# InternetMaximalism/plonky2_bn254

Measured on AMD Instinct MI355X. Metric: G1 scalar-mul STARK proofs/sec (256-bit scalars), higher is better.
Workload: dtype u64 (Goldilocks p = 2^64-2^32+1; BN254 Fq as 10x26-bit Montgomery limbs); 1 GPU; configs[1]: batch of 1024 G1 scalar-muls on 1 GPU per step = 8 proofs x 128 instances, 2^16 rows, W=781, standard_fast_config; instances_per_proof=128, steps_in_flight=4, parallelism=1 GPU, no collective

## Files before the change

include/bn254_stark.h:

```cpp
#ifndef BN254_STARK_H
#define BN254_STARK_H

#include <stddef.h>
#include <stdint.h>

#ifdef __cplusplus
extern "C" {
#endif

#define BN254S_ABI_VERSION 1

enum {
  BN254S_OK = 0,
  BN254S_E_INVALID_ARG = -1,
  BN254S_E_HIP = -2,
  BN254S_E_OOM = -3,
  BN254S_E_INVALID_POINT = -4,
  BN254S_E_UNSUPPORTED = -5,
  BN254S_E_TRANSCRIPT = -6,
  BN254S_E_INTERNAL = -7,
  BN254S_E_VERIFY = -8
};

typedef struct bn254s_ctx bn254s_ctx;
// ... 143 lines not shown
int bn254s_job_outputs_batch(bn254s_ctx* ctx, int kind, const uint64_t* scalars , const uint64_t* x,
                             const uint64_t* offset, size_t n, uint64_t* outputs_out ,
                             uint8_t* finite_out );
int bn254s_job_outputs(bn254s_ctx* ctx, int kind, const bn254s_params* params, const uint64_t* scalars, const uint64_t* x,
                       const uint64_t* offset, size_t n, size_t per_proof, uint64_t* outputs_out, bn254s_proof** proofs_out);
int bn254s_commit_values(bn254s_ctx* ctx, const uint64_t* values, size_t ncols, uint64_t* coeffs, uint64_t* lde,
                         uint64_t* cap);
int bn254s_bench_ntt(bn254s_ctx* ctx, size_t ncols, int iters, float* ms);
int bn254s_bench_ntt_clock(bn254s_ctx* ctx, size_t ncols, int iters, float* ms, float* mhz, float* mhz_min);
int bn254s_bench_issue(bn254s_ctx* ctx, float* ns_per_issue, float* mhz);
int bn254s_bench_copy(bn254s_ctx* ctx, size_t words, int iters);
int bn254s_bench_leafhash(bn254s_ctx* ctx, size_t ncols, int log_leaves, int iters, float* ms);
int bn254s_poseidon_permute(bn254s_ctx* ctx, uint64_t* states, size_t n);
int bn254s_selftest_field(bn254s_ctx* ctx, const uint64_t* a, const uint64_t* b, size_t n, uint64_t* out);
int bn254s_selftest_poseidon(bn254s_ctx* ctx, int variant, uint64_t* states, size_t n);
int bn254s_selftest_leaf_hash(bn254s_ctx* ctx, const uint64_t* data, size_t ncols, int log_leaves, int kernel, int chunk_cols,
                              uint64_t* digests);
int bn254s_selftest_fq_inv(bn254s_ctx* ctx, const uint64_t* x, size_t n, uint64_t* out);
int bn254s_selftest_fq(bn254s_ctx* ctx, int group, const uint64_t* in, size_t n, uint64_t* out);
int bn254s_selftest_logup(bn254s_ctx* ctx, const uint64_t* trace, size_t rows, int ncols, int rc_begin, int n_rc, int table_col,
                          int freq_col, const uint64_t betas[2], uint64_t* out);
int bn254s_selftest_acc(bn254s_ctx* ctx, const uint64_t* values, const uint64_t* weights, size_t T, size_t rows, uint64_t* out);
int bn254s_selftest_openings(bn254s_ctx* ctx, const uint64_t* coeffs, int npolys, int log_r, const uint64_t zeta[2],
                             const uint64_t zeta_next[2], uint64_t* out);
int bn254s_selftest_fri_combine(bn254s_ctx* ctx, int mode, int W, int n_rc, int n_ctl, size_t n, const uint64_t* cols,
                                const uint64_t* aux_in, const uint64_t* points, uint64_t* out);
int bn254s_selftest_fri_fold(bn254s_ctx* ctx, const uint64_t* in, int log_m, uint64_t shift, const uint64_t beta[2], uint64_t* out);
int bn254s_selftest_fri_rows(bn254s_ctx* ctx, const uint64_t* lde, int ncols, int log_n, int h, size_t k0, size_t rows,
                             const uint32_t* indices, int nq, uint64_t* window, uint64_t* gathered);
int bn254s_selftest_transforms(bn254s_ctx* ctx, int op, int log_n, int flags, int ncols, int coset_mask, const uint64_t* in,
                               uint64_t* out0, uint64_t* out1);
int bn254s_selftest_mul_2exp(bn254s_ctx* ctx, const uint64_t* x, size_t n, uint64_t* out);
int bn254s_selftest_outer_dft(bn254s_ctx* ctx, int log_r, int inverse, const uint64_t* in, size_t n, uint64_t* out);
#define BN254S_VERIFY_RECORD_HEAD 34
int bn254s_selftest_verify_front(int kind, const bn254s_params* params, uint32_t degree_bits, const uint64_t* words, size_t n_words,
                                 uint64_t* record_out, size_t record_cap);
int bn254s_selftest_query_round(bn254s_ctx* ctx, int kind, const bn254s_params* params, uint32_t degree_bits,
                                const uint64_t* const* words, size_t n_words, const uint64_t* records, size_t n_proofs,
                                size_t chunk_proofs, int32_t* codes_out);
const char* bn254s_selftest_query_text(int n_layers, int code);
int bn254s_selftest_verify_batch_ms(bn254s_ctx* ctx, float ms_out[5]);
#define BN254S_PLAN_WORDS 54
int bn254s_selftest_proof_plan(int kind, size_t n, const bn254s_params* params, uint64_t dev_total_bytes, int force_split,
                               int force_lowmem, int force_stream, int stream_win_log, uint64_t* out, char* err, size_t err_len);
int bn254s_generate_trace(bn254s_ctx* ctx, int kind, const uint64_t* scalars, const uint64_t* x, const uint64_t* offset,
                          size_t n, uint32_t min_rows_log2, uint64_t* trace_out, uint64_t* outputs);
int bn254s_g1_generate_trace(bn254s_ctx* ctx, const uint64_t* scalars, const uint64_t* x, const uint64_t* offset,
                             size_t n, uint32_t min_rows_log2, uint64_t* trace_out, uint64_t* outputs);

#ifdef __cplusplus
}
#endif
#endif
```

plonky2_bn254_amd/csrc/ctx.h:

```cpp
#pragma once
#include <string>
#include <vector>
#include <map>
#include <cstdio>
#include <mutex>
#include <condition_variable>
#include <chrono>
#include <deque>
#include <functional>
#include <thread>
#include <atomic>
#include <hip/hip_runtime.h>
#include "../../include/bn254_stark.h"
#include "gl_dev.h"
#include "ntt.h"

struct BufPool {
  std::map<std::string, std::pair<void*, size_t>> pool;
  std::string err;
  void* buf(const std::string& name, size_t bytes) {
    auto it = pool.find(name);
    if (it != pool.end() && it->second.second >= bytes) return it->second.first;
    if (it != pool.end()) {
      hipFree(it->second.first);
      pool.erase(it);
    }
    void* p = nullptr;
    if (hipMalloc(&p, bytes) != hipSuccess) {
      (void)hipGetLastError();
      err = "hipMalloc failed for " + name + " (" + std::to_string(bytes) + " bytes)";
      return nullptr;
    }
    pool[name] = {p, bytes};
    return p;
  }
  u64* words(const std::string& name, size_t n) { return (u64*)buf(name, n * 8); }
  bool has(const std::string& name) const { return pool.find(name) != pool.end(); }
  void drop(const std::string& name) {
    auto it = pool.find(name);
    if (it == pool.end()) return;
    hipFree(it->second.first);
    pool.erase(it);
  }
  void release() {
    for (auto& kv : pool) hipFree(kv.second.first);
    pool.clear();
  }
};

struct Slot {
  hipStream_t st = nullptr;
  BufPool mem;
  void* pinned = nullptr;
  size_t pinned_bytes = 0;
  std::vector<hipEvent_t> events;
};

enum { BIG_NTT = 0, BIG_EXCL = 1, BIG_HASH = 2, BIG_HASH_PART = 3 };

struct WorkPool {
  std::mutex mu;
  std::condition_variable cv, done_cv;
  std::deque<std::function<void(size_t)>> q;
  std::vector<std::thread> th;
  std::vector<char> busy;
  bool stop = false;
  size_t limit = 0, n_busy = 0;
  size_t n_waiting = 0, completions = 0;
  std::mutex retry_mu;
  std::atomic<int> in_flight{0};
  void start(size_t n, int device) {
    std::lock_guard<std::mutex> lk(mu);
    limit = n;
    if (busy.size() < n) busy.resize(n, 0);
    while (th.size() < n) {
      th.emplace_back([this, device]() {
        (void)hipSetDevice(device);
        for (;;) {
          std::function<void(size_t)> f;
          size_t s = 0;
          {
            std::unique_lock<std::mutex> lk2(mu);
            auto free_slot = [&]() -> size_t {
              for (size_t i = 0; i < limit && i < busy.size(); i++)
                if (!busy[i]) return i;
              return (size_t)-1;
            };
            cv.wait(lk2, [&] { return (stop && q.empty()) || (!q.empty() && n_busy < limit && free_slot() != (size_t)-1); });
            if (q.empty()) return;
            f = std::move(q.front());
            q.pop_front();
// ... 36 lines not shown
    }
    for (size_t i : idle) g(i);
    {
      std::lock_guard<std::mutex> lk(mu);
      for (size_t i : idle) busy[i] = 0;
    }
    cv.notify_all();
  }
  size_t active() {
    std::lock_guard<std::mutex> lk(mu);
    return n_busy - n_waiting;
  }
  size_t completions_now() {
    std::lock_guard<std::mutex> lk(mu);
    return completions;
  }
  void wait_for_a_completion(size_t c0) {
    std::unique_lock<std::mutex> lk(mu);
    n_waiting++;
    done_cv.wait_for(lk, std::chrono::seconds(60), [&] { return completions != c0; });
    n_waiting--;
  }
  void shutdown() {
    {
      std::lock_guard<std::mutex> lk(mu);
      stop = true;
    }
    cv.notify_all();
    for (auto& t : th) t.join();
    th.clear();
  }
};

struct bn254s_ctx : BufPool {
  int device = 0;
  hipStream_t stream = nullptr;
  NttTables ntt;
  std::vector<Slot*> slots;
  WorkPool workers;
  std::mutex plans_mu;
  std::map<std::pair<unsigned, bool>, NttPlan> plans;
  const NttPlan* ntt_plan(unsigned log_n, bool split) {
    std::lock_guard<std::mutex> lk(plans_mu);
    const auto key = std::make_pair(log_n, split);
    auto it = plans.find(key);
    if (it != plans.end()) return &it->second;
    NttPlan p;
    if (ntt_plan_init(&p, &ntt, log_n, split) != 0) return nullptr;
    return &(plans[key] = p);
  }
  std::mutex big_mu;
  std::condition_variable big_cv;
  int big_cap = 12, big_cost[4] = {12, 2, 4, 2}, big_used = 0;
  int hash_split = 1;
  bool big_fifo = true;
  struct BigWaiter {
    unsigned long id;
    int cls;
  };
  std::deque<BigWaiter> big_q;
  unsigned long big_next_id = 0;
  int big_convoy = 4, big_convoy_run = 0;
  bool big_last_was_ntt = false;
  void big_lock(int cls) {
    std::unique_lock<std::mutex> lk(big_mu);
    if (big_fifo) {
      const unsigned long my = big_next_id++;
      big_q.push_back({my, cls});
      big_cv.wait(lk, [&] {
        if (big_q.front().id == my) {
          if (big_used + big_cost[cls] > big_cap) return false;
          if (big_last_was_ntt && cls != BIG_NTT && big_convoy_run < big_convoy)
            for (const BigWaiter& w : big_q)
              if (w.cls == BIG_NTT) return false;
          return true;
        }
        if (cls != BIG_NTT || !big_last_was_ntt || big_used != 0 || big_convoy_run >= big_convoy) return false;
        if (big_q.front().cls == BIG_NTT) return false;
        for (const BigWaiter& w : big_q) {
          if (w.cls == BIG_NTT) return w.id == my;
        }
        return false;
      });
      const bool in_order = big_q.front().id == my;
      for (auto it = big_q.begin(); it != big_q.end(); ++it)
        if (it->id == my) {
          big_q.erase(it);
          break;
        }
      if (in_order) big_convoy_run = 0;
      else big_convoy_run++;
      big_last_was_ntt = false;
      big_used += big_cost[cls];
      lk.unlock();
      big_cv.notify_all();
      return;
    }
    big_cv.wait(lk, [&] { return big_used + big_cost[cls] <= big_cap; });
    big_used += big_cost[cls];
  }
  void big_unlock(int cls) {
    {
      std::lock_guard<std::mutex> lk(big_mu);
      big_used -= big_cost[cls];
      big_last_was_ntt = cls == BIG_NTT && big_used == 0;
    }
    big_cv.notify_all();
  }
  static constexpr size_t MAX_SLOTS = 64;
  std::mutex slots_mu, err_mu;
  float vb_ms[5] = {0, 0, 0, 0, 0};
  bn254s_ctx() { slots.reserve(MAX_SLOTS); }
  void set_err(const std::string& e) {
    std::lock_guard<std::mutex> lk(err_mu);
    err = e;
  }
  size_t n_slots_now() {
    std::lock_guard<std::mutex> lk(slots_mu);
    return slots.size();
  }
  Slot* slot(size_t i) {
    if (i >= MAX_SLOTS) return nullptr;
    std::lock_guard<std::mutex> lk(slots_mu);
    while (slots.size() <= i) {
      Slot* s = new Slot();
      if (hipStreamCreateWithFlags(&s->st, hipStreamNonBlocking) != hipSuccess) {
        delete s;
        return nullptr;
      }
      slots.push_back(s);
    }
    return slots[i];
  }
};

#define HIP_TRY(ctx, call)                                                                  \
  do {                                                                                      \
    hipError_t e_ = (call);                                                                 \
    if (e_ != hipSuccess) {                                                                 \
      (ctx)->set_err(std::string(#call) + ": " + hipGetErrorString(e_));                    \
      return BN254S_E_HIP;                                                                  \
// ... 3 lines not shown
```

plonky2_bn254_amd/csrc/ntt.h:

```cpp
#pragma once
#include <vector>
#include "gl_dev.h"

static constexpr size_t NTT_N = 65536;

struct NttTables {
  u64 *tw256_fwd = nullptr, *tw256_inv = nullptr;
  u64 *twmat_fwd = nullptr, *twmat_inv = nullptr;
  u64* twmat_inv_ninv = nullptr;
  u64* coset_pow[2] = {nullptr, nullptr};
  u64* coset_inv_pow[2] = {nullptr, nullptr};
  u64 n_inv = 0;
};

int ntt_tables_init(NttTables* T);
void ntt_tables_free(NttTables* T);

struct NttTallTables {
  unsigned log_n = 0;
  u64* wn_inv_pow = nullptr;
  u64* wn_pow_br = nullptr;
  u64* block_coset_pow[2] = {nullptr, nullptr};
  u64 shift[2] = {0, 0};
  u64 r_inv = 0;
};
struct NttSplitTables {
  unsigned log_n = 0;
  u64 *fwd_lo = nullptr, *fwd_hi = nullptr, *inv_lo = nullptr, *inv_hi = nullptr;
  u64 shift[2] = {0, 0};
  u64 half = 0;
};

struct NttPlan {
  unsigned log_n = 0, log_s = 0, log_r = 0;
  const NttTables* base = nullptr;
  NttTallTables tall;
  NttSplitTables split;
};
int ntt_plan_init(NttPlan* P, const NttTables* base, unsigned log_n, bool split);
void ntt_plan_free(NttPlan* P);
size_t ntt_scratch_words(unsigned log_n, bool split, int ncols);
void ntt_commit(const NttPlan& P, const u64* vals, u64* coef, u64* lde, size_t lde_stride, u64* scratch, int ncols, hipStream_t s);
void ntt_lde(const NttPlan& P, const u64* coef, u64* lde, size_t lde_stride, u64* scratch, int ncols, hipStream_t s, int coset_mask = 3);
void ntt_coset_inverse(const NttPlan& P, int h, const u64* vals, u64* coef, u64* scratch, int ncols, hipStream_t s);

static constexpr int FIELD_SELFTEST_OUTS = 17;
void field_selftest(const u64* a, const u64* b, u64* out, size_t n, hipStream_t s);
void mul_2exp_selftest(const u64* x, u64* out, size_t n, hipStream_t s);
void outer_dft_selftest(int log_r, bool inverse, const u64* in, u64* out, size_t n, hipStream_t s);
```

plonky2_bn254_amd/csrc/ntt.hip:

```cpp
#include <cassert>
#include <type_traits>
#include "gl_dev.h"
#include "gl_asm.h"
#include "ntt.h"

#if defined(__HIP_DEVICE_COMPILE__) && defined(BN254S_NTT_PRIO) && BN254S_NTT_PRIO > 0
#define NTT_KERNEL_PRIO() __builtin_amdgcn_s_setprio(BN254S_NTT_PRIO)
#else
#define NTT_KERNEL_PRIO() ((void)0)
#endif

template <bool INV, int SPAN, int G, int J>
__device__ __forceinline__ void bfly16(u64* x) {
  constexpr int E = J * (8 / SPAN);
  constexpr int S0 = E == 0 ? 0 : (!INV ? 12 * E : 192 - 12 * E);
  constexpr bool NEG0 = S0 >= 96;
  constexpr int S1 = NEG0 ? S0 - 96 : S0;
  constexpr bool RIGHT = S1 > 64;
  constexpr bool NEG = NEG0 != RIGHT;
  u64 s, d;
  gl_bfly_asm<NEG>(x[G + J], x[G + J + SPAN], s, d);
  x[G + J] = s;
  if constexpr (S1 == 0) x[G + J + SPAN] = d;
  else if constexpr (RIGHT) x[G + J + SPAN] = gl_shr_small_asm<96 - S1>(d);
// ... 618 lines not shown
  k_coset_unscale_half<<<dim3((unsigned)(H / 256), 2 * ncols), 256, 0, s>>>(coeffs, H, TT->log_n - 16, gl_mul(si, si));
}

int ntt_plan_init(NttPlan* P, const NttTables* base, unsigned log_n, bool split) {
  *P = NttPlan{};
  if (log_n < 16 || log_n - split > 22 || (split && log_n < 18)) return -1;
  P->log_n = log_n;
  P->log_s = split ? 1 : 0;
  P->log_r = log_n - 16 - P->log_s;
  P->base = base;
  if ((P->log_r && tall_tables_init(&P->tall, log_n - P->log_s, split ? gl_mul(GL_GEN, GL_GEN) : GL_GEN)) ||
      (split && split_tables_init(&P->split, log_n))) {
    ntt_plan_free(P);
    return -1;
  }
  return 0;
}
void ntt_plan_free(NttPlan* P) {
  tall_tables_free(&P->tall);
  split_tables_free(&P->split);
}
size_t ntt_scratch_words(unsigned log_n, bool split, int ncols) { return (size_t)(log_n == 16 || split ? 3 : 1) * ncols << log_n; }

void ntt_commit(const NttPlan& P, const u64* vals, u64* coef, u64* lde, size_t lde_stride, u64* scratch, int ncols, hipStream_t s) {
  const size_t N = (size_t)1 << P.log_n;
  assert(P.log_s || lde_stride == 2 * N);
  if (P.log_s) {
    split_inverse(&P.split, vals, coef, ncols, s);
    commit_tall(P.base, &P.tall, coef, coef, scratch, scratch + (size_t)ncols * 2 * N, 2 * ncols, s);
    split_forward(&P.split, scratch, lde, lde_stride, ncols, s, 3);
  } else if (P.log_r) commit_tall(P.base, &P.tall, vals, coef, lde, scratch, ncols, s);
  else commit_base(P.base, vals, coef, lde, scratch, ncols, s);
}
void ntt_lde(const NttPlan& P, const u64* coef, u64* lde, size_t lde_stride, u64* scratch, int ncols, hipStream_t s, int coset_mask) {
  const size_t N = (size_t)1 << P.log_n;
  assert(P.log_s || lde_stride == 2 * N);
  assert(P.log_r || coset_mask == 3);
  if (P.log_s) {
    lde_tall(P.base, &P.tall, coef, scratch, scratch + (size_t)ncols * 2 * N, 2 * ncols, s, coset_mask);
    split_forward(&P.split, scratch, lde, lde_stride, ncols, s, coset_mask);
  } else if (P.log_r) lde_tall(P.base, &P.tall, coef, lde, scratch, ncols, s, coset_mask);
  else lde_base(P.base, coef, lde, scratch, ncols, s);
}
void ntt_coset_inverse(const NttPlan& P, int h, const u64* vals, u64* coef, u64* scratch, int ncols, hipStream_t s) {
  if (P.log_s) coset_inverse_split(P.base, &P.tall, &P.split, h, vals, coef, scratch, ncols, s);
  else if (P.log_r) coset_inverse_tall(P.base, &P.tall, h, vals, coef, scratch, ncols, s);
  else coset_inverse_base(P.base, h, vals, coef, scratch, ncols, s);
}

__global__ void k_field_selftest(const u64* __restrict__ a, const u64* __restrict__ b, u64* __restrict__ out, size_t n) {
  size_t i = (size_t)blockIdx.x * blockDim.x + threadIdx.x;
  if (i >= n) return;
  const u64 x = a[i], y = b[i];
  u64* o = out + i * FIELD_SELFTEST_OUTS;
  u64 s, d, s2, d2;
  gl_bfly_asm<false>(x, y, s, d);
  gl_bfly_asm<true>(x, y, s2, d2);
  o[0] = s;
  o[1] = d;
  o[2] = d2;
  o[3] = s2 == s ? gl_mul_asm(x, y) : ~0ull;
  o[4] = gl_shl_asm<12>(x);
  o[5] = gl_shl_asm<24>(x);
  o[6] = gl_shl_asm<32>(x);
  o[7] = gl_shl_asm<36>(x);
  o[8] = gl_shl_asm<48>(x);
// ... 49 lines not shown
```

plonky2_bn254_amd/csrc/ntt_selftest.hip:

```cpp
#include "ctx.h"
#include "transforms.h"

static bool all_canonical(const uint64_t* w, size_t n) {
  for (size_t k = 0; k < n; k++)
    if (w[k] >= GL_P) return false;
  return true;
}

extern "C" {

int bn254s_selftest_transforms(bn254s_ctx* c, int op, int log_n, int flags, int ncols, int coset_mask, const uint64_t* in,
                               uint64_t* out0, uint64_t* out1) {
  if (!c || !in || !out0 || (op == 0 && !out1)) return BN254S_E_INVALID_ARG;
  if (op < 0 || op > 3 || log_n < 16 || log_n > 23 || flags < 0 || flags > 3 || ncols < 1 || ncols > 64) return BN254S_E_INVALID_ARG;
  const bool split = flags & 1, compact = flags & 2;
  if ((split && log_n < 18) || (!split && log_n == 23) || (compact && log_n == 16)) return BN254S_E_INVALID_ARG;
  if (op == 2 && (log_n == 16 || ncols > Transforms::CH || coset_mask < 1 || coset_mask > 3)) return BN254S_E_INVALID_ARG;
  if (op == 3 && ncols != 2 * 2) return BN254S_E_INVALID_ARG;
  if (op == 1 && compact && !split && ncols > Transforms::CH) return BN254S_E_INVALID_ARG;
  ProofPlan pl;
  pl.log_n = (unsigned)log_n;
  const size_t N = pl.N = (size_t)1 << log_n, M2 = pl.M2 = 2 * N;
  pl.log_m2 = pl.log_n + 1;
  pl.log_s = split ? 1 : 0;
// ... 2 lines not shown
  if (!all_canonical(in, n_in)) return BN254S_E_INVALID_ARG;

  HIP_TRY(c, hipSetDevice(c->device));
  const NttPlan* np = c->ntt_plan(pl.log_n, split);
  if (!np) {
    c->set_err("NTT tables");
    return BN254S_E_OOM;
  }
  const size_t n_lde = (size_t)ncols * M2;
  u64* d_in = c->words("ns.in", n_in);
  u64* d_coef = op == 0 || op == 3 ? c->words("ns.coef", n_in) : nullptr;
  u64* d_lde = op != 3 ? c->words("ns.lde", n_lde) : nullptr;
  u64* d_tmp = c->words("ns.tmp", pl.ntt_tmp_words(ncols));
  if (!d_in || !d_tmp || (!d_coef && (op == 0 || op == 3)) || (!d_lde && op != 3)) return BN254S_E_OOM;
  hipStream_t st = c->stream;
  HIP_TRY(c, hipMemcpyAsync(d_in, in, 8 * n_in, hipMemcpyHostToDevice, st));
  const Transforms tf{*np, st, pl, d_tmp, d_lde, nullptr};
  switch (op) {
    case 0: tf.commit_ntt(d_in, d_coef, d_lde, ncols); break;
    case 1: tf.lde(d_in, d_lde, ncols); break;
    case 2:
      HIP_TRY(c, hipMemsetAsync(d_lde, 0xFF, 8 * n_lde, st));
      tf.lde_chunk(d_in, ncols, coset_mask);
      break;
    default: tf.quotient_coset_inverse(d_in, d_coef); break;
  }
  HIP_TRY(c, hipGetLastError());
  if (op == 0 || op == 3) HIP_TRY(c, hipMemcpyAsync(out0, d_coef, 8 * n_in, hipMemcpyDeviceToHost, st));
  if (op != 3) HIP_TRY(c, hipMemcpyAsync(op == 0 ? out1 : out0, d_lde, 8 * n_lde, hipMemcpyDeviceToHost, st));
  HIP_TRY(c, hipStreamSynchronize(st));
  return BN254S_OK;
}

int bn254s_selftest_mul_2exp(bn254s_ctx* c, const uint64_t* x, size_t n, uint64_t* out) {
  if (!c || !x || !out || n < 1 || n > ((size_t)1 << 20) || !all_canonical(x, n)) return BN254S_E_INVALID_ARG;
  HIP_TRY(c, hipSetDevice(c->device));
  u64* d = c->words("ns.shift", n + 64 * n);
  if (!d) return BN254S_E_OOM;
  HIP_TRY(c, hipMemcpyAsync(d, x, 8 * n, hipMemcpyHostToDevice, c->stream));
  mul_2exp_selftest(d, d + n, n, c->stream);
  HIP_TRY(c, hipGetLastError());
  HIP_TRY(c, hipMemcpyAsync(out, d + n, 8 * 64 * n, hipMemcpyDeviceToHost, c->stream));
  HIP_TRY(c, hipStreamSynchronize(c->stream));
  return BN254S_OK;
}

int bn254s_selftest_outer_dft(bn254s_ctx* c, int log_r, int inverse, const uint64_t* in, size_t n, uint64_t* out) {
  if (!c || !in || !out || log_r < 1 || log_r > 6 || inverse < 0 || inverse > 1 || n < 1 || n > ((size_t)1 << 16)) return BN254S_E_INVALID_ARG;
  const size_t words = n << log_r;
  if (!all_canonical(in, words)) return BN254S_E_INVALID_ARG;
  HIP_TRY(c, hipSetDevice(c->device));
  u64* d = c->words("ns.dft", 2 * words);
  if (!d) return BN254S_E_OOM;
  HIP_TRY(c, hipMemcpyAsync(d, in, 8 * words, hipMemcpyHostToDevice, c->stream));
  outer_dft_selftest(log_r, inverse != 0, d, d + words, n, c->stream);
  HIP_TRY(c, hipGetLastError());
  HIP_TRY(c, hipMemcpyAsync(out, d + words, 8 * words, hipMemcpyDeviceToHost, c->stream));
  HIP_TRY(c, hipStreamSynchronize(c->stream));
  return BN254S_OK;
}

}
```

plonky2_bn254_amd/csrc/prover.hip:

```cpp
#include <algorithm>
#include <atomic>
#include <cstring>
#include <thread>
#include "ctx.h"
#include "trace.h"
#include "aux.h"
#include "merkle.h"
#include "quotient.h"
#include "fri.h"
#include "transcript.h"
#include "prover.h"
#include "proof_plan.h"
#include "transforms.h"

template <class L>
static StarkShape make_shape(bool input_has_a, int n_constraints) {
  StarkShape s;
  s.W = L::W;
  s.rc_begin = L::RC_BEGIN;
  s.rc_end = L::RC_END;
  s.table_col = L::RANGE;
  s.freq_col = L::FREQ;
  s.n_ctl = 2;
  s.n_constraints = n_constraints;
// ... 251 lines not shown
  CHK(hipMemsetAsync(ws.err, 0, 16, st));
  u64* d_outs = ws.open;
  if (int rc = upload_and_generate(stark_kind(pl.kind), scalars, x, off, pl.n, ws.in, ws.tvals, pl.N, ws.scr, d_outs, ws.err, st, false, err))
    return rc;
  {
    BigSection big(r.c, st, BIG_EXCL);
    launch_range_columns(ws.tvals, pl.N, sh.rc_begin, sh.rc_end, sh.freq_col, sh.table_col, (u32*)ws.hist, ws.err, st);
  }
  pr->outputs.resize(pl.n * (size_t)pl.PW);
  CHK(hipMemcpyAsync(pr->outputs.data(), d_outs, pl.n * (size_t)pl.PW * 8, hipMemcpyDeviceToHost, st));
  CHK(hipMemcpyAsync(h_err, ws.err, 4, hipMemcpyDeviceToHost, st));
  r.se(ST_TRACE);
  return BN254S_OK;
}

static void hash_sections(const Run& r, const u64* lde, int width, u64* tree, int stage) {
  bn254s_ctx* c = r.c;
  const size_t M2 = r.pl.M2;
  const int S = r.pl.log_n == 16 ? c->hash_split : 1;
  if (S <= 1) {
    BigSection big(c, r.st, BIG_HASH);
    r.sb(stage);
    merkle_leaves(lde, 1, M2, width, r.pl.log_m2, tree, r.st);
    return;
  }
  const size_t cnt = M2 / S;
  for (int k = 0; k < S; k++) {
    BigSection big(c, r.st, BIG_HASH_PART);
    if (k == 0) r.sb(stage);
    merkle_leaves_range(lde, 1, M2, width, (size_t)k * cnt, cnt, tree, r.st);
  }
}

static int commit(const Run& r, const u64* vals, u64* coef, u64* lde, int width, u64* tree, int ntt_stage, int merkle_stage,
                  u64* cap_out, std::string& err) {
  const ProofPlan& pl = r.pl;
  hipStream_t st = r.st;
  if (pl.stream) {
    BigSection big(r.c, st, BIG_NTT);
    r.sb(ntt_stage);
    r.tf.commit_stream(vals, coef, width, tree);
    r.se(ntt_stage);
    r.sb(merkle_stage);
  } else {
    {
      BigSection big(r.c, st, BIG_NTT);
      r.sb(ntt_stage);
      r.tf.commit_ntt(vals, coef, lde, width);
      r.se(ntt_stage);
    }
    hash_sections(r, lde, width, tree, merkle_stage);
  }
  merkle_upper(pl.log_m2, pl.P.cap_height, tree, st, r.mmode());
  CHK(hipMemcpyAsync(cap_out, tree + r.ws.cap_off, ProofPlan::CAPW * 8, hipMemcpyDeviceToHost, st));
  r.se(merkle_stage);
  CHK(hipStreamSynchronize(st));
  return BN254S_OK;
}

static void stage_aux(const Run& r, const u64 betas[2], const u64 gammas[2]) {
  BigSection big(r.c, r.st, BIG_EXCL);
  r.sb(ST_AUX);
  aux_build(r.pl.sh, r.ws.tvals, r.pl.N, betas, gammas, r.ws.avals, r.ws.scr, r.ws.err, r.st);
  r.se(ST_AUX);
}

static void quotient_over_windows(const Run& r, const u64 betas[2], const u64 gammas[2]) {
  const ProofPlan& pl = r.pl;
  const Workspace& ws = r.ws;
  hipStream_t st = r.st;
  const size_t N = pl.N, M2 = pl.M2, BK = pl.BK, WROWS = pl.WROWS;
  BigSection big(r.c, st, BIG_NTT);
  r.sb(ST_QUOTIENT);
  QPointTables wpt;
  wpt.x = ws.wpt;
  wpt.lfirst = ws.wpt + WROWS;
  wpt.llast = ws.wpt + 2 * WROWS;
  for (int h = 0; h < 2; h++)
// ... 725 lines not shown
```

plonky2_bn254_amd/lib.py:

```python
from __future__ import annotations

import ctypes as C
import os
from typing import Optional

import numpy as np

_HERE = os.path.dirname(os.path.abspath(__file__))
LIB_PATH = os.environ.get("BN254S_LIB") or os.path.join(_HERE, "libbn254stark.so")

U64P = C.POINTER(C.c_uint64)


class LibraryMissing(RuntimeError):
    pass


class VerifyError(RuntimeError):
    """bn254s_verify rejected the proof; the message is the reference verifier's error text."""


class Params(C.Structure):
    _fields_ = [(n, C.c_uint32) for n in (
        "struct_size", "security_bits", "num_challenges", "rate_bits", "cap_height", "pow_bits",
# ... 71 lines not shown
    lib.bn254s_hash_to_g2_batch.argtypes = [vp, vp, C.c_size_t, C.c_size_t, vp]
    lib.bn254s_job_outputs_batch.argtypes = [vp, C.c_int, vp, vp, vp, C.c_size_t, vp, vp]
    lib.bn254s_job_outputs.argtypes = [vp, C.c_int, C.POINTER(Params), vp, vp, vp, C.c_size_t, C.c_size_t, vp, C.POINTER(vp)]
    lib.bn254s_hash_to_fq2_batch.argtypes = [vp, vp, C.c_size_t, C.c_size_t, vp]
    if hasattr(lib, "bn254s_map_to_g1"):
        lib.bn254s_hash_to_fq.argtypes = [vp, C.c_size_t, vp]
        lib.bn254s_hash_to_fq_batch.argtypes = [vp, vp, C.c_size_t, C.c_size_t, vp]
        lib.bn254s_map_to_g1_batch.argtypes = [vp, vp, C.c_size_t, vp, vp, vp]
        lib.bn254s_hash_to_g1_batch.argtypes = [vp, vp, C.c_size_t, C.c_size_t, vp]
        lib.bn254s_map_to_g1.argtypes = [vp, C.POINTER(Params), vp, C.c_size_t, C.c_size_t, vp, vp, vp, C.POINTER(vp)]
    lib.bn254s_ctl_values.argtypes = [C.c_int, vp, vp, vp, vp, C.c_size_t, vp, vp]
    lib.bn254s_commit_values.argtypes = [vp, vp, C.c_size_t, vp, vp, vp]
    lib.bn254s_bench_ntt.argtypes = [vp, C.c_size_t, C.c_int, C.POINTER(C.c_float)]
    lib.bn254s_bench_ntt_clock.argtypes = [vp, C.c_size_t, C.c_int, C.POINTER(C.c_float), C.POINTER(C.c_float), C.POINTER(C.c_float)]
    lib.bn254s_bench_issue.argtypes = [vp, C.POINTER(C.c_float), C.POINTER(C.c_float)]
    lib.bn254s_poseidon_permute.argtypes = [vp, vp, C.c_size_t]
    lib.bn254s_selftest_field.argtypes = [vp, vp, vp, C.c_size_t, vp]
    lib.bn254s_selftest_poseidon.argtypes = [vp, C.c_int, vp, C.c_size_t]
    lib.bn254s_selftest_leaf_hash.argtypes = [vp, vp, C.c_size_t, C.c_int, C.c_int, C.c_int, vp]
    lib.bn254s_selftest_fq_inv.argtypes = [vp, vp, C.c_size_t, vp]
    lib.bn254s_selftest_fq.argtypes = [vp, C.c_int, vp, C.c_size_t, vp]
    if hasattr(lib, "bn254s_selftest_logup"):
        lib.bn254s_selftest_logup.argtypes = [vp, vp, C.c_size_t, C.c_int, C.c_int, C.c_int, C.c_int, C.c_int, vp, vp]
    if hasattr(lib, "bn254s_selftest_fri_fold"):
        lib.bn254s_selftest_acc.argtypes = [vp, vp, vp, C.c_size_t, C.c_size_t, vp]
        lib.bn254s_selftest_openings.argtypes = [vp, vp, C.c_int, C.c_int, vp, vp, vp]
        lib.bn254s_selftest_fri_combine.argtypes = [vp, C.c_int, C.c_int, C.c_int, C.c_int, C.c_size_t, vp, vp, vp, vp]
        lib.bn254s_selftest_fri_fold.argtypes = [vp, vp, C.c_int, C.c_uint64, vp, vp]
        lib.bn254s_selftest_fri_rows.argtypes = [vp, vp, C.c_int, C.c_int, C.c_int, C.c_size_t, C.c_size_t, vp, C.c_int, vp, vp]
    if hasattr(lib, "bn254s_selftest_transforms"):
        lib.bn254s_selftest_transforms.argtypes = [vp, C.c_int, C.c_int, C.c_int, C.c_int, C.c_int, vp, vp, vp]
        lib.bn254s_selftest_mul_2exp.argtypes = [vp, vp, C.c_size_t, vp]
        lib.bn254s_selftest_outer_dft.argtypes = [vp, C.c_int, C.c_int, vp, C.c_size_t, vp]
    if hasattr(lib, "bn254s_selftest_proof_plan"):
        lib.bn254s_selftest_proof_plan.argtypes = [C.c_int, C.c_size_t, C.POINTER(Params), C.c_uint64, C.c_int, C.c_int, C.c_int,
                                                   C.c_int, vp, C.c_char_p, C.c_size_t]
    lib.bn254s_bench_copy.argtypes = [vp, C.c_size_t, C.c_int]
    lib.bn254s_bench_leafhash.argtypes = [vp, C.c_size_t, C.c_int, C.c_int, C.POINTER(C.c_float)]
    lib.bn254s_g1_generate_trace.argtypes = [vp, vp, vp, vp, C.c_size_t, C.c_uint32, vp, vp]
    _lib = lib
    return lib


def default_params() -> Params:
    p = Params()
    load_library().bn254s_params_default(C.byref(p))
    return p


def _ptr(a: Optional[np.ndarray]):
    if a is None:
        return None
    assert a.dtype == np.uint64 and a.flags["C_CONTIGUOUS"]
    return a.ctypes.data_as(C.c_void_p)


def _slots(n_jobs, per_proof):
    return (C.c_void_p * ((n_jobs + per_proof - 1) // per_proof))()


def _proofs(lib, slots):
    return [Proof(lib, C.c_void_p(h)) for h in slots]


class Proof:

# ... 505 lines not shown
    def selftest_fri_fold(self, vals: np.ndarray, shift: int, beta) -> np.ndarray:
        vals = np.ascontiguousarray(vals, dtype=np.uint64)
        m = vals.shape[0]
        assert vals.shape == (m, 2) and m >= 16 and m & (m - 1) == 0
        b = np.array([int(beta[0]), int(beta[1])], dtype=np.uint64)
        out = np.zeros((m >> 4, 2), np.uint64)
        self._check(self._lib.bn254s_selftest_fri_fold(self._h, _ptr(vals), m.bit_length() - 1, int(shift), _ptr(b), _ptr(out)),
                    "bn254s_selftest_fri_fold")
        return out

    def selftest_fri_rows(self, lde: np.ndarray, h: int, k0: int, rows: int, indices):
        lde = np.ascontiguousarray(lde, dtype=np.uint64)
        ncols, m2 = lde.shape
        assert m2 >= 4 and m2 & (m2 - 1) == 0
        idx = np.ascontiguousarray(indices, dtype=np.uint32)
        win = np.zeros((ncols, rows), np.uint64)
        gat = np.zeros((ncols, idx.shape[0]), np.uint64)
        self._check(self._lib.bn254s_selftest_fri_rows(self._h, _ptr(lde), ncols, m2.bit_length() - 2, h, k0, rows,
                                                       idx.ctypes.data_as(C.c_void_p), idx.shape[0], _ptr(win), _ptr(gat)),
                    "bn254s_selftest_fri_rows")
        return win, gat

    TRANSFORM_SPLIT, TRANSFORM_COMPACT = 1, 2

    def selftest_transforms(self, op: int, log_n: int, flags: int, data: np.ndarray, coset_mask: int = 3):
        data = np.ascontiguousarray(data, dtype=np.uint64)
        ncols, n = data.shape
        assert n == 1 << log_n, (n, log_n)
        out0 = np.zeros((ncols, n if op in (0, 3) else 2 * n), np.uint64)
        out1 = np.zeros((ncols, 2 * n), np.uint64) if op == 0 else None
        self._check(self._lib.bn254s_selftest_transforms(self._h, op, log_n, flags, ncols, coset_mask, _ptr(data), _ptr(out0),
                                                         _ptr(out1)), "bn254s_selftest_transforms")
        return (out0, out1) if op == 0 else out0

    def selftest_mul_2exp(self, x: np.ndarray) -> np.ndarray:
        x = np.ascontiguousarray(x, dtype=np.uint64)
        out = np.zeros((x.shape[0], 64), np.uint64)
        self._check(self._lib.bn254s_selftest_mul_2exp(self._h, _ptr(x), x.shape[0], _ptr(out)), "bn254s_selftest_mul_2exp")
        return out

    def selftest_outer_dft(self, log_r: int, inverse: bool, rows: np.ndarray) -> np.ndarray:
        rows = np.ascontiguousarray(rows, dtype=np.uint64)
        assert rows.ndim == 2 and rows.shape[1] == 1 << log_r, (rows.shape, log_r)
        out = np.zeros_like(rows)
        self._check(self._lib.bn254s_selftest_outer_dft(self._h, log_r, int(inverse), _ptr(rows), rows.shape[0], _ptr(out)),
                    "bn254s_selftest_outer_dft")
        return out

    def poseidon_permute(self, states: np.ndarray) -> np.ndarray:
        st = np.ascontiguousarray(states, dtype=np.uint64).copy()
        self._check(self._lib.bn254s_poseidon_permute(self._h, _ptr(st), st.shape[0]), "bn254s_poseidon_permute")
        return st

    def generate_trace(self, kind, scalars, x, offset=None, min_rows_log2=16):
        width, pw = {0: (781, 8), 1: (1295, 16), 2: (427, 4)}[kind]
        n = scalars.shape[0]
        rows = max(1 << min_rows_log2, 512 * n)
        rows = 1 << (rows - 1).bit_length()
        trace = np.zeros((width, rows), np.uint64)
        outs = np.zeros((n, pw), np.uint64)
        self._check(self._lib.bn254s_generate_trace(self._h, kind, _ptr(scalars), _ptr(x), _ptr(offset), n, min_rows_log2,
                                                    _ptr(trace), _ptr(outs)), "bn254s_generate_trace")
        return trace, outs

    def g1_generate_trace(self, scalars, x, offset, min_rows_log2=16, width=781):
        n = scalars.shape[0]
# ... 485 lines not shown
```

Baseline: 91.15 proofs/s.

## Batch queued NTT commit jobs into one exclusive big-section on a single stream

```diff
diff --git a/include/bn254_stark.h b/include/bn254_stark.h
--- a/include/bn254_stark.h
+++ b/include/bn254_stark.h
@@ -199,6 +199,8 @@
                                uint64_t* out0, uint64_t* out1);
 int bn254s_selftest_mul_2exp(bn254s_ctx* ctx, const uint64_t* x, size_t n, uint64_t* out);
 int bn254s_selftest_outer_dft(bn254s_ctx* ctx, int log_r, int inverse, const uint64_t* in, size_t n, uint64_t* out);
+int bn254s_selftest_commit_batch(bn254s_ctx* ctx, int njobs, const int* ncols, const uint64_t* in, uint64_t* coef_out,
+                                 uint64_t* lde_out, uint64_t sections_out[3]);
 #define BN254S_VERIFY_RECORD_HEAD 34
 int bn254s_selftest_verify_front(int kind, const bn254s_params* params, uint32_t degree_bits, const uint64_t* words, size_t n_words,
                                  uint64_t* record_out, size_t record_cap);
diff --git a/plonky2_bn254_amd/csrc/big_queue.h b/plonky2_bn254_amd/csrc/big_queue.h
--- /dev/null
+++ b/plonky2_bn254_amd/csrc/big_queue.h
@@ -0,0 +1,149 @@
+#pragma once
+#include <condition_variable>
+#include <deque>
+#include <mutex>
+
+enum { BIG_NTT = 0, BIG_EXCL = 1, BIG_HASH = 2, BIG_HASH_PART = 3 };
+
+struct BigQueue {
+  std::mutex big_mu;
+  std::condition_variable big_cv;
+  int big_cap = 12, big_cost[4] = {12, 2, 4, 2}, big_used = 0;
+  int hash_split = 1;
+  bool big_fifo = true;
+  static constexpr int BIG_SECTION_JOBS = 8;
+  enum { W_WAITING = 0, W_CLAIMED, W_DONE };
+  struct BigWaiter {
+    unsigned long id;
+    int cls;
+    void* job;
+    int state, status;
+    int overtaken;
+  };
+  std::deque<BigWaiter*> big_q;
+  unsigned long big_next_id = 0;
+  int big_convoy = 4, big_convoy_run = 0;
+  bool big_last_was_ntt = false;
+  unsigned long long big_stat_sections = 0, big_stat_stages = 0, big_stat_largest = 0;
+  int big_stat_overtaken = 0;
+
+  bool big_admissible(const BigWaiter& w) const {
+    const int cls = w.cls;
+    if (big_q.front() == &w) {
+      if (big_used + big_cost[cls] > big_cap) return false;
+      if (big_last_was_ntt && cls != BIG_NTT && big_convoy_run < big_convoy)
+        for (const BigWaiter* o : big_q)
+          if (o->cls == BIG_NTT) return false;
+      return true;
+    }
+    if (cls != BIG_NTT || !big_last_was_ntt || big_used != 0 || big_convoy_run >= big_convoy) return false;
+    if (big_q.front()->cls == BIG_NTT) return false;
+    for (const BigWaiter* o : big_q)
+      if (o->cls == BIG_NTT) return o == &w;
+    return false;
+  }
+  void big_dequeue(BigWaiter* w) {
+    const bool in_order = big_q.front() == w;
+    for (auto it = big_q.begin(); it != big_q.end(); ++it)
+      if (*it == w) {
+        big_q.erase(it);
+        break;
+      }
+    if (in_order) big_convoy_run = 0;
+    else {
+      big_convoy_run++;
+      if (++big_q.front()->overtaken > big_stat_overtaken) big_stat_overtaken = big_q.front()->overtaken;
+    }
+  }
+  BigWaiter* big_next_in_convoy() const {
+    if (big_q.empty()) return nullptr;
+    if (big_q.front()->cls == BIG_NTT) return big_q.front();
+    if (big_convoy_run >= big_convoy) return nullptr;
+    for (BigWaiter* o : big_q)
+      if (o->cls == BIG_NTT) return o;
+    return nullptr;
+  }
+  bool big_wait(std::unique_lock<std::mutex>& lk, BigWaiter& w) {
+    if (!big_fifo) {
+      big_cv.wait(lk, [&] { return big_used + big_cost[w.cls] <= big_cap; });
+      big_used += big_cost[w.cls];
+      return true;
+    }
+    w.id = big_next_id++;
+    big_q.push_back(&w);
+    big_cv.wait(lk, [&] { return w.state == W_DONE || (w.state == W_WAITING && big_admissible(w)); });
+    if (w.state == W_DONE) return false;
+    big_dequeue(&w);
+    big_last_was_ntt = false;
+    big_used += big_cost[w.cls];
+    return true;
+  }
+  void big_lock(int cls) {
+    BigWaiter w{0, cls, nullptr, W_WAITING, 0, 0};
+    {
+      std::unique_lock<std::mutex> lk(big_mu);
+      big_wait(lk, w);
+      if (cls == BIG_NTT) {
+        big_stat_sections++;
+        big_stat_stages++;
+        if (big_stat_largest < 1) big_stat_largest = 1;
+      }
+    }
+    big_cv.notify_all();
+  }
+  void big_unlock(int cls) {
+    {
+      std::lock_guard<std::mutex> lk(big_mu);
+      big_used -= big_cost[cls];
+      big_last_was_ntt = cls == BIG_NTT && big_used == 0;
+    }
+    big_cv.notify_all();
+  }
+  template <class Run>
+  int big_ntt_section(void* job, Run&& run) {
+    BigWaiter me{0, BIG_NTT, job, W_WAITING, 0, 0};
+    BigWaiter* grp[BIG_SECTION_JOBS];
+    int n = 0;
+    {
+      std::unique_lock<std::mutex> lk(big_mu);
+      if (!big_wait(lk, me)) return me.status;
+      grp[n++] = &me;
+      if (big_fifo && big_convoy > 0 && big_cost[BIG_NTT] >= big_cap)
+        while (n < BIG_SECTION_JOBS) {
+          BigWaiter* w = big_next_in_convoy();
+          if (!w || !w->job) break;
+          big_dequeue(w);
+          w->state = W_CLAIMED;
+          grp[n++] = w;
+        }
+      big_stat_sections++;
+      big_stat_stages += (unsigned long long)n;
+      if (big_stat_largest < (unsigned long long)n) big_stat_largest = (unsigned long long)n;
+    }
+    big_cv.notify_all();
+    void* jobs[BIG_SECTION_JOBS];
+    int status[BIG_SECTION_JOBS];
+    for (int i = 0; i < n; i++) {
+      jobs[i] = grp[i]->job;
+      status[i] = 0;
+    }
+    run(jobs, n, status);
+    {
+      std::lock_guard<std::mutex> lk(big_mu);
+      big_used -= big_cost[BIG_NTT];
+      big_last_was_ntt = big_used == 0;
+      for (int i = 1; i < n; i++) {
+        grp[i]->status = status[i];
+        grp[i]->state = W_DONE;
+      }
+    }
+    big_cv.notify_all();
+    return status[0];
+  }
+  void big_stats(unsigned long long out[3]) {
+    std::lock_guard<std::mutex> lk(big_mu);
+    out[0] = big_stat_sections;
+    out[1] = big_stat_stages;
+    out[2] = big_stat_largest;
+  }
+};
diff --git a/plonky2_bn254_amd/csrc/ctx.h b/plonky2_bn254_amd/csrc/ctx.h
--- a/plonky2_bn254_amd/csrc/ctx.h
+++ b/plonky2_bn254_amd/csrc/ctx.h
@@ -14,6 +14,7 @@
 #include "../../include/bn254_stark.h"
 #include "gl_dev.h"
 #include "ntt.h"
+#include "big_queue.h"
 
 struct BufPool {
   std::map<std::string, std::pair<void*, size_t>> pool;
@@ -55,8 +56,6 @@
   size_t pinned_bytes = 0;
   std::vector<hipEvent_t> events;
 };
-
-enum { BIG_NTT = 0, BIG_EXCL = 1, BIG_HASH = 2, BIG_HASH_PART = 3 };
 
 struct WorkPool {
   std::mutex mu;
@@ -159,7 +158,7 @@
   }
 };
 
-struct bn254s_ctx : BufPool {
+struct bn254s_ctx : BufPool, BigQueue {
   int device = 0;
   hipStream_t stream = nullptr;
   NttTables ntt;
@@ -176,64 +175,6 @@
     if (ntt_plan_init(&p, &ntt, log_n, split) != 0) return nullptr;
     return &(plans[key] = p);
   }
-  std::mutex big_mu;
-  std::condition_variable big_cv;
-  int big_cap = 12, big_cost[4] = {12, 2, 4, 2}, big_used = 0;
-  int hash_split = 1;
-  bool big_fifo = true;
-  struct BigWaiter {
-    unsigned long id;
-    int cls;
-  };
-  std::deque<BigWaiter> big_q;
-  unsigned long big_next_id = 0;
-  int big_convoy = 4, big_convoy_run = 0;
-  bool big_last_was_ntt = false;
-  void big_lock(int cls) {
-    std::unique_lock<std::mutex> lk(big_mu);
-    if (big_fifo) {
-      const unsigned long my = big_next_id++;
-      big_q.push_back({my, cls});
-      big_cv.wait(lk, [&] {
-        if (big_q.front().id == my) {
-          if (big_used + big_cost[cls] > big_cap) return false;
-          if (big_last_was_ntt && cls != BIG_NTT && big_convoy_run < big_convoy)
-            for (const BigWaiter& w : big_q)
-              if (w.cls == BIG_NTT) return false;
-          return true;
-        }
-        if (cls != BIG_NTT || !big_last_was_ntt || big_used != 0 || big_convoy_run >= big_convoy) return false;
-        if (big_q.front().cls == BIG_NTT) return false;
-        for (const BigWaiter& w : big_q) {
-          if (w.cls == BIG_NTT) return w.id == my;
-        }
-        return false;
-      });
-      const bool in_order = big_q.front().id == my;
-      for (auto it = big_q.begin(); it != big_q.end(); ++it)
-        if (it->id == my) {
-          big_q.erase(it);
-          break;
-        }
-      if (in_order) big_convoy_run = 0;
-      else big_convoy_run++;
-      big_last_was_ntt = false;
-      big_used += big_cost[cls];
-      lk.unlock();
-      big_cv.notify_all();
-      return;
-    }
-    big_cv.wait(lk, [&] { return big_used + big_cost[cls] <= big_cap; });
-    big_used += big_cost[cls];
-  }
-  void big_unlock(int cls) {
-    {
-      std::lock_guard<std::mutex> lk(big_mu);
-      big_used -= big_cost[cls];
-      big_last_was_ntt = cls == BIG_NTT && big_used == 0;
-    }
-    big_cv.notify_all();
-  }
   static constexpr size_t MAX_SLOTS = 64;
   std::mutex slots_mu, err_mu;
   float vb_ms[5] = {0, 0, 0, 0, 0};
diff --git a/plonky2_bn254_amd/csrc/ntt.h b/plonky2_bn254_amd/csrc/ntt.h
--- a/plonky2_bn254_amd/csrc/ntt.h
+++ b/plonky2_bn254_amd/csrc/ntt.h
@@ -41,6 +41,15 @@
 void ntt_plan_free(NttPlan* P);
 size_t ntt_scratch_words(unsigned log_n, bool split, int ncols);
 void ntt_commit(const NttPlan& P, const u64* vals, u64* coef, u64* lde, size_t lde_stride, u64* scratch, int ncols, hipStream_t s);
+struct NttCommitJob {
+  const NttPlan* plan;
+  const u64* vals;
+  u64 *coef, *lde, *scratch;
+  int ncols;
+  hipEvent_t ev_begin, ev_end;
+  int status;
+};
+void ntt_commit_batch(NttCommitJob* const* jobs, int n, hipStream_t s);
 void ntt_lde(const NttPlan& P, const u64* coef, u64* lde, size_t lde_stride, u64* scratch, int ncols, hipStream_t s, int coset_mask = 3);
 void ntt_coset_inverse(const NttPlan& P, int h, const u64* vals, u64* coef, u64* scratch, int ncols, hipStream_t s);
 
diff --git a/plonky2_bn254_amd/csrc/ntt.hip b/plonky2_bn254_amd/csrc/ntt.hip
--- a/plonky2_bn254_amd/csrc/ntt.hip
+++ b/plonky2_bn254_amd/csrc/ntt.hip
@@ -674,6 +674,16 @@
   } else if (P.log_r) commit_tall(P.base, &P.tall, vals, coef, lde, scratch, ncols, s);
   else commit_base(P.base, vals, coef, lde, scratch, ncols, s);
 }
+void ntt_commit_batch(NttCommitJob* const* jobs, int n, hipStream_t s) {
+  for (int i = 0; i < n; i++) {
+    NttCommitJob& j = *jobs[i];
+    assert(j.plan->log_r == 0 && j.plan->log_s == 0);
+    if (j.ev_begin) (void)hipEventRecord(j.ev_begin, s);
+    commit_base(j.plan->base, j.vals, j.coef, j.lde, j.scratch, j.ncols, s);
+    j.status = (int)hipGetLastError();
+    if (j.ev_end) (void)hipEventRecord(j.ev_end, s);
+  }
+}
 void ntt_lde(const NttPlan& P, const u64* coef, u64* lde, size_t lde_stride, u64* scratch, int ncols, hipStream_t s, int coset_mask) {
   const size_t N = (size_t)1 << P.log_n;
   assert(P.log_s || lde_stride == 2 * N);
diff --git a/plonky2_bn254_amd/csrc/ntt_selftest.hip b/plonky2_bn254_amd/csrc/ntt_selftest.hip
--- a/plonky2_bn254_amd/csrc/ntt_selftest.hip
+++ b/plonky2_bn254_amd/csrc/ntt_selftest.hip
@@ -58,6 +58,49 @@
   return BN254S_OK;
 }
 
+int bn254s_selftest_commit_batch(bn254s_ctx* c, int njobs, const int* ncols, const uint64_t* in, uint64_t* coef_out, uint64_t* lde_out,
+                                 uint64_t sections_out[3]) {
+  if (!c || njobs < 0 || njobs > BigQueue::BIG_SECTION_JOBS) return BN254S_E_INVALID_ARG;
+  if (njobs && (!ncols || !in || !coef_out || !lde_out)) return BN254S_E_INVALID_ARG;
+  size_t total = 0;
+  for (int j = 0; j < njobs; j++) {
+    if (ncols[j] < 1 || ncols[j] > 64) return BN254S_E_INVALID_ARG;
+    total += (size_t)ncols[j];
+  }
+  if (njobs) {
+    const size_t N = NTT_N;
+    if (!all_canonical(in, total * N)) return BN254S_E_INVALID_ARG;
+    HIP_TRY(c, hipSetDevice(c->device));
+    const NttPlan* np = c->ntt_plan(16, false);
+    u64* d_in = c->words("ns.in", total * N);
+    u64* d_coef = c->words("ns.coef", total * N);
+    u64* d_lde = c->words("ns.lde", total * 2 * N);
+    u64* d_tmp = c->words("ns.tmp", ntt_scratch_words(16, false, (int)total));
+    if (!np || !d_in || !d_coef || !d_lde || !d_tmp) return BN254S_E_OOM;
+    hipStream_t st = c->stream;
+    HIP_TRY(c, hipMemcpyAsync(d_in, in, 8 * total * N, hipMemcpyHostToDevice, st));
+    NttCommitJob jobs[BigQueue::BIG_SECTION_JOBS];
+    NttCommitJob* tb[BigQueue::BIG_SECTION_JOBS];
+    size_t c0 = 0;
+    for (int j = 0; j < njobs; j++) {
+      jobs[j] = NttCommitJob{np, d_in + c0 * N, d_coef + c0 * N, d_lde + c0 * 2 * N, d_tmp + c0 * 3 * N, ncols[j], nullptr, nullptr, 0};
+      tb[j] = &jobs[j];
+      c0 += (size_t)ncols[j];
+    }
+    ntt_commit_batch(tb, njobs, st);
+    for (int j = 0; j < njobs; j++) HIP_TRY(c, (hipError_t)jobs[j].status);
+    HIP_TRY(c, hipMemcpyAsync(coef_out, d_coef, 8 * total * N, hipMemcpyDeviceToHost, st));
+    HIP_TRY(c, hipMemcpyAsync(lde_out, d_lde, 8 * total * 2 * N, hipMemcpyDeviceToHost, st));
+    HIP_TRY(c, hipStreamSynchronize(st));
+  }
+  if (sections_out) {
+    unsigned long long s[3];
+    c->big_stats(s);
+    for (int k = 0; k < 3; k++) sections_out[k] = s[k];
+  }
+  return BN254S_OK;
+}
+
 int bn254s_selftest_mul_2exp(bn254s_ctx* c, const uint64_t* x, size_t n, uint64_t* out) {
   if (!c || !x || !out || n < 1 || n > ((size_t)1 << 20) || !all_canonical(x, n)) return BN254S_E_INVALID_ARG;
   HIP_TRY(c, hipSetDevice(c->device));
diff --git a/plonky2_bn254_amd/csrc/prover.hip b/plonky2_bn254_amd/csrc/prover.hip
--- a/plonky2_bn254_amd/csrc/prover.hip
+++ b/plonky2_bn254_amd/csrc/prover.hip
@@ -307,6 +307,26 @@
   }
 }
 
+static int ntt_section_base(const Run& r, const u64* vals, u64* coef, u64* lde, int width, int ntt_stage, std::string& err) {
+  hipStream_t st = r.st;
+  CHK(hipStreamSynchronize(st));
+  NttCommitJob job{&r.tf.np, vals, coef, lde, r.tf.tmp, width, r.sl.events[2 * ntt_stage], r.sl.events[2 * ntt_stage + 1], 0};
+  const int rc = r.c->big_ntt_section(&job, [st](void* const* jobs, int n, int* status) {
+    const hipError_t own = hipGetLastError();
+    NttCommitJob* tb[BigQueue::BIG_SECTION_JOBS];
+    for (int i = 0; i < n; i++) tb[i] = static_cast<NttCommitJob*>(jobs[i]);
+    ntt_commit_batch(tb, n, st);
+    const hipError_t done = hipStreamSynchronize(st);
+    for (int i = 0; i < n; i++) status[i] = done != hipSuccess ? (int)done : tb[i]->status;
+    if (own != hipSuccess) status[0] = (int)own;
+  });
+  if (rc != 0) {
+    err = std::string("NTT stage: ") + hipGetErrorString((hipError_t)rc);
+    return BN254S_E_HIP;
+  }
+  return BN254S_OK;
+}
+
 static int commit(const Run& r, const u64* vals, u64* coef, u64* lde, int width, u64* tree, int ntt_stage, int merkle_stage,
                   u64* cap_out, std::string& err) {
   const ProofPlan& pl = r.pl;
@@ -318,7 +338,9 @@
     r.se(ntt_stage);
     r.sb(merkle_stage);
   } else {
-    {
+    if (pl.log_n == 16 && !pl.lowmem) {
+      if (int rc = ntt_section_base(r, vals, coef, lde, width, ntt_stage, err)) return rc;
+    } else {
       BigSection big(r.c, st, BIG_NTT);
       r.sb(ntt_stage);
       r.tf.commit_ntt(vals, coef, lde, width);
diff --git a/plonky2_bn254_amd/lib.py b/plonky2_bn254_amd/lib.py
--- a/plonky2_bn254_amd/lib.py
+++ b/plonky2_bn254_amd/lib.py
@@ -127,6 +127,8 @@
         lib.bn254s_selftest_transforms.argtypes = [vp, C.c_int, C.c_int, C.c_int, C.c_int, C.c_int, vp, vp, vp]
         lib.bn254s_selftest_mul_2exp.argtypes = [vp, vp, C.c_size_t, vp]
         lib.bn254s_selftest_outer_dft.argtypes = [vp, C.c_int, C.c_int, vp, C.c_size_t, vp]
+    if hasattr(lib, "bn254s_selftest_commit_batch"):
+        lib.bn254s_selftest_commit_batch.argtypes = [vp, C.c_int, vp, vp, vp, vp, vp]
     if hasattr(lib, "bn254s_selftest_proof_plan"):
         lib.bn254s_selftest_proof_plan.argtypes = [C.c_int, C.c_size_t, C.POINTER(Params), C.c_uint64, C.c_int, C.c_int, C.c_int,
                                                    C.c_int, vp, C.c_char_p, C.c_size_t]
@@ -698,6 +700,23 @@
         self._check(self._lib.bn254s_selftest_transforms(self._h, op, log_n, flags, ncols, coset_mask, _ptr(data), _ptr(out0),
                                                          _ptr(out1)), "bn254s_selftest_transforms")
         return (out0, out1) if op == 0 else out0
+
+    def selftest_commit_batch(self, jobs):
+        jobs = [np.ascontiguousarray(j, dtype=np.uint64) for j in jobs]
+        assert jobs and all(j.ndim == 2 and j.shape[1] == 65536 for j in jobs)
+        ncols = np.array([j.shape[0] for j in jobs], dtype=np.int32)
+        data = np.ascontiguousarray(np.concatenate(jobs, axis=0))
+        coef = np.zeros_like(data)
+        lde = np.zeros((data.shape[0], 2 * 65536), np.uint64)
+        self._check(self._lib.bn254s_selftest_commit_batch(self._h, len(jobs), ncols.ctypes.data_as(C.c_void_p), _ptr(data), _ptr(coef),
+                                                           _ptr(lde), None), "bn254s_selftest_commit_batch")
+        ends = np.cumsum(ncols)
+        return [(coef[e - n:e], lde[e - n:e]) for e, n in zip(ends, ncols)]
+
+    def ntt_section_counters(self):
+        out = np.zeros(3, np.uint64)
+        self._check(self._lib.bn254s_selftest_commit_batch(self._h, 0, None, None, None, None, _ptr(out)), "bn254s_selftest_commit_batch")
+        return tuple(int(v) for v in out)
 
     def selftest_mul_2exp(self, x: np.ndarray) -> np.ndarray:
         x = np.ascontiguousarray(x, dtype=np.uint64)
```

New measurement: 91.82 proofs/s (median of 6 runs). About the same (+0.7%).
